# aki-k-no/gaussian-splatting-npu

Hardware: AMD Instinct MI355X
Metric: rendered Mpix/s fwd+bwd, 1M Gaussians @1080p (higher is better)
Workload: dtype f32; 1 GPU; BASELINE config 4: 8 views per step of config 2 (1000000 Gaussians, SH deg 3, 1920x1080, fwd+bwd each), view v on rank v mod 1, grads accumulated on one GPU; P=1000000, width=1920, height=1080, views_per_rank=8, antialiasing=False, parallelism=views-dp1, forward_views_reruns=1

## Files before the change

### gaussian-splatting-npu_amd/csrc/capi.hip

```cpp
#include <stdio.h>
#include <stdlib.h>
#include <string.h>

#include <string>
#include <vector>

#include "gsr.h"
#include "simple_knn.h"
#include "fused_ssim.h"
#include "gsr_common.h"
#include "gsr_kernels.h"

using namespace gsr;

static_assert(GSR_ACC_MEANS3D == ACC_MEANS3D && GSR_ACC_DC == ACC_DC && GSR_ACC_SH == ACC_SH &&
                  GSR_ACC_OPACITY == ACC_OPACITY && GSR_ACC_SCALES == ACC_SCALES &&
                  GSR_ACC_ROTATIONS == ACC_ROTATIONS && GSR_ACC_COV3D == ACC_COV3D && GSR_ACC_COLORS == ACC_COLORS,
              "include/gsr.h accumulate bits match the kernel's");

namespace {

thread_local std::string g_err;
thread_local uint32_t* g_pinned = nullptr;
constexpr uint32_t L_PENDING = 0xFFFFFFFFu;
constexpr int GSR_RERUN_WIDE = -100;
thread_local int t_last_depth_passes[MAX_VIEWS] = {};
// ... 27 lines not shown
    } while (0)

constexpr int PINNED_SLOT_WORDS = 16;
int pinned(int slot, uint32_t** out)
{
    if (!g_pinned) {
        hipError_t e = hipHostMalloc((void**)&g_pinned, 4 * PINNED_SLOT_WORDS * (MAX_VIEWS + 2),
                                     hipHostMallocMapped | hipHostMallocCoherent);
        if (e != hipSuccess) return fail_hip(e, __LINE__);
    }
    *out = g_pinned + PINNED_SLOT_WORDS * slot;
    return GSR_OK;
}

constexpr unsigned EVENT_FLAGS = hipEventDisableTiming | hipEventDisableSystemFence;
struct PrefixStream {
    hipStream_t s = nullptr;
    hipEvent_t in = nullptr, out = nullptr;
};
constexpr int MAX_DEVICES = 64;
thread_local PrefixStream g_prefix[MAX_DEVICES];
thread_local PrefixStream g_aux[MAX_DEVICES];
thread_local int g_prefix_mode = 1;

int stream_fork(PrefixStream* streams, bool on, hipStream_t from, hipStream_t* out)
{
    *out = from;
    if (!on) return GSR_OK;
    int dev = 0;
    HIP_TRY(hipGetDevice(&dev));
    if (dev < 0 || dev >= MAX_DEVICES) return GSR_OK;
    PrefixStream& ps = streams[dev];
    if (!ps.s) {
        int least = 0, greatest = 0;
        HIP_TRY(hipDeviceGetStreamPriorityRange(&least, &greatest));
        HIP_TRY(hipEventCreateWithFlags(&ps.in, EVENT_FLAGS));
        HIP_TRY(hipEventCreateWithFlags(&ps.out, EVENT_FLAGS));
        HIP_TRY(hipStreamCreateWithPriority(&ps.s, hipStreamNonBlocking, greatest));
    }
    HIP_TRY(hipEventRecord(ps.in, from));
    HIP_TRY(hipStreamWaitEvent(ps.s, ps.in, 0));
    *out = ps.s;
    return GSR_OK;
}

int stream_join(PrefixStream* streams, hipStream_t from, hipStream_t forked)
// ... 77 lines not shown
struct Camera {
    const float *view, *proj, *campos;
    float tan_fovx, tan_fovy;
};
struct ViewState {
    char *geometry, *image, *binning;
    size_t binning_capacity;
    float *out_color, *invdepth;
    int* radii;
};

}

extern "C" {

const char* gsr_last_error(void) { return g_err.c_str(); }

const char* gsr_version(void) { return GSR_REF_ALPHA ? "gsr-hip 0.1 gfx950 ref-alpha (TEST BUILD)" : "gsr-hip 0.1 gfx950"; }

int gsr_set_prefix_stream(int on)
{
    if (on < 0 || on > 2) return fail(GSR_ERR_INVALID, "prefix stream mode must be 0, 1 or 2");
    g_prefix_mode = on;
    return GSR_OK;
}

int gsr_profile_enable(int on)
{
    g_prof.on = on != 0;
    for (int k = 0; k < PK_COUNT; k++) g_prof.used[k] = 0;
    return PK_COUNT;
}

const char* gsr_profile_kernel_name(int k) { return (k >= 0 && k < PK_COUNT) ? kProfNames[k] : ""; }

int gsr_profile_read(double* total_ms, int* counts, int n)
{
    for (int k = 0; k < PK_COUNT && k < n; k++) {
        double acc = 0.0;
        for (size_t j = 0; j < g_prof.used[k]; j++) {
            auto& ev = g_prof.pool[k][j];
            HIP_TRY(hipEventSynchronize(ev.second));
            float ms = 0.f;
            HIP_TRY(hipEventElapsedTime(&ms, ev.first, ev.second));
            acc += ms;
        }
// ... 286 lines not shown
    TileHistJob hj[MAX_VIEWS];
    OrderJob dj[MAX_VIEWS];
    for (int v = 0; v < V; v++) {
        char* gb = vs[v].geometry;
        const PreprocessArgs& a = pa[v];
        rec[v] = {a.tiles_touched, at<uint32_t>(gb, g.off[GEOM_EMIT_START]), P, a.scan_status + scan_status_words(P),
                  nullptr};
        dsort[v] = depth_sort_job(gb, a, hdev[v]);
        uint32_t* offsets = at<uint32_t>(gb, g.off[GEOM_POINT_OFFSETS]);
        off[v] = {offsets, offsets, P, a.scan_status, hdev[v] + 2};
        hj[v] = {a.rect4, P, a.tile_diff};
        dj[v] = diff_order_job(vs[v].image, sc.width, sc.height);
    }
    hipStream_t aux = ps;
    int rc = stream_fork(g_aux, g_prefix_mode != 0, ps, &aux);
    if (rc) return rc;
    hipError_t e = launch_scan_batch(rec, V, true, aux);
    if (e == hipSuccess && use_tile_diff(tg.gx, tg.gy)) {
        ProfScope ps_(PK_RANGES, aux);
        e = launch_tile_hist_batch(hj, V, tg.gx, tg.gy, aux);
    }
    if (e == hipSuccess && use_tile_diff(tg.gx, tg.gy)) {
        ProfScope ps_(PK_TILE_ORDER, aux);
        e = launch_tile_order_batch(dj, V, tg.T, aux);
    }
    if (e == hipSuccess) {
        ProfScope ps_(PK_DEPTH_SORT, ps);
        e = radix_sort_batch(dsort, V, DEPTH_BITS, ps);
    }
    if (e == hipSuccess) {
        ProfScope ps_(PK_SCAN, ps);
        e = launch_scan_batch(off, V, false, ps);
    }
    rc = stream_join(g_aux, ps, aux);
    if (e != hipSuccess) return fail_hip(e, __LINE__);
    if (rc) return rc;
    if (opt.early_count) {
        int all[MAX_VIEWS];
        for (int v = 0; v < V; v++) all[v] = v;
        rc = tile_sort_count_pass(sc, vs, all, V, ps);
        if (rc) return rc;
    }
    DEBUG_SYNC(ps);
    int wide[MAX_VIEWS], nw = 0;
    for (int v = 0; v < V && !rc; v++) {
        rc = forward_geometry_wait(h[v], ps, &L[v]);
        t_last_depth_passes[v] = depth_force_wide() ? 4 : 3;
// ... 18 lines not shown
    }
    if (rc)
        for (int v = 0; v < V; v++) L[v] = 0;
    return rc;
}

static int forward_render(const Scene& sc, const ViewState* vs, const int* L, const int* which, int n,
                          const float* background, bool counted, hipStream_t caller, hipStream_t ps, bool debug)
{
    const TileGrid tg(sc.width, sc.height);
    const ImageLayout im = image_layout(sc.width, sc.height);
    TileSortJob tsort[MAX_VIEWS];
    RangesJob rj[MAX_VIEWS];
    OrderJob oj[MAX_VIEWS];
    RenderFwdArgs ra[MAX_VIEWS];
    int ns = 0;
    for (int k = 0; k < n; k++) {
        const ViewState& s = vs[which[k]];
        const int Lv = L[which[k]];
        if (Lv > 0) tsort[ns++] = fused_tile_sort_job(sc, s, Lv, false);
        uint2* ranges = at<uint2>(s.image, im.off[IMG_RANGES]);
        rj[k] = {Lv, Lv > 0 ? at<uint32_t>(s.binning, bin_layout(Lv).off[BIN_SORTED_TILES]) : nullptr, ranges};
        oj[k] = {ranges, nullptr, at<uint32_t>(s.image, im.off[IMG_TILE_ORDER])};
        ra[k] = render_fwd_args(sc, s, Lv, background);
    }
    if (ns) {
        ProfScope ps_(PK_TILE_SORT, ps, counted);
        HIP_TRY(tile_sort_fused_batch(tsort, ns, tg.gx, tg.T, ps, counted ? FUSED_SCATTER : FUSED_ALL));
    }
    DEBUG_SYNC(ps);
    if (n && !use_tile_diff(tg.gx, tg.gy)) {
        {
            ProfScope ps_(PK_RANGES, ps);
            HIP_TRY(launch_tile_ranges_batch(rj, n, tg.T, ps));
        }
        DEBUG_SYNC(ps);
        ProfScope ps_(PK_TILE_ORDER, ps);
        HIP_TRY(launch_tile_order_batch(oj, n, tg.T, ps));
    }
    DEBUG_SYNC(ps);
    const int rc = stream_join(g_prefix, caller, ps);
    if (rc) return rc;
    if (n) {
        ProfScope ps_(PK_RENDER_FWD, caller);
        HIP_TRY(launch_render_fwd_batch(ra, n, tg.T, caller));
    }
    DEBUG_SYNC(caller);
    return GSR_OK;
}

static bool binning_fits(const ViewState& vs, int L)
{
    return vs.binning && gsr_binning_buffer_size(L) <= vs.binning_capacity;
}

int gsr_forward_geometry_dc(char* geometry_buffer, char* image_buffer, int P, int D, int M, int width, int height,
                         const float* means3D, const float* dc, const float* shs, const float* colors_precomp,
                         const float* opacities, const float* scales, float scale_modifier,
                         const float* rotations, const float* cov3D_precomp, const float* viewmatrix,
                         const float* projmatrix, const float* cam_pos, float tan_fovx, float tan_fovy,
                         bool prefiltered, bool antialiasing, int* radii, bool debug, gsr_stream_t stream,
// ... 160 lines not shown
    r.T = tg.T;
    r.bg = background;
    r.splat = at<float4>(gb, g.off[GEOM_SPLAT]);
    r.final_Ts = at<float>(ib, im.off[IMG_FINAL_T]);
    r.n_contrib = at<uint32_t>(ib, im.off[IMG_N_CONTRIB]);
    r.dL_dpixels = dL_dpix;
    r.dL_invdepths = dL_invdepths;
    r.grad_inst = at<float>(bb, b.off[BIN_GRAD_INST]);
    r.slot = slots_from_rect(tg.gx, tg.gy) ? nullptr : at<uint32_t>(bb, b.off[BIN_SLOT]);
    r.valid = at<uint32_t>(bb, b.off[BIN_VALID]);
    r.hit = at<uint8_t>(bb, b.off[BIN_HIT]);
    r.emit_start = at<uint32_t>(gb, g.off[GEOM_EMIT_START]);
    r.rec_mask = at<uint32_t>(gb, g.off[GEOM_REC_MASK]);
    return r;
}

static int backward_render_impl(const Scene& sc, const ViewState& vs, int R, const float* background,
                                const float* dL_dpix, const float* dL_invdepths, bool debug, hipStream_t s)
{
    const ImageLayout im = image_layout(sc.width, sc.height);
    const RenderBwdArgs r = render_bwd_args(sc, vs, R, background, dL_dpix, dL_invdepths);
    {
        ProfScope ps_(PK_TILE_ORDER, s);
        HIP_TRY(launch_tile_order(nullptr, r.tile_work, r.T, at<uint32_t>(vs.image, im.off[IMG_TILE_ORDER]), s));
    }
    {
        ProfScope ps_(PK_RENDER_BWD, s);
        HIP_TRY(launch_render_bwd(r, r.T, s));
    }
    DEBUG_SYNC(s);
    return GSR_OK;
}

static int preprocess_bwd_shared(PreprocessBwdArgs& p, const Scene& sc, bool has_invdepth, float* dL_dcolor,
                                 float* dL_dopacity, float* dL_dmean3D, float* dL_dcov3D, float* dL_ddc,
                                 float* dL_dsh, float* dL_dscale, float* dL_drot, unsigned accumulate)
{
    if (accumulate & ~(unsigned)GSR_ACC_ALL) return fail(GSR_ERR_INVALID, "unknown accumulate bits");
    if (sc.dc && !dL_ddc) return fail(GSR_ERR_INVALID, "dc given without dL_ddc");
    if (sc.dc && sc.colors_precomp)
        return fail(GSR_ERR_INVALID, "Please provide exactly one of either SHs or precomputed colors!");
    if (sc.dc && sc.M > 0 && (!sc.shs || !dL_dsh))
        return fail(GSR_ERR_INVALID, "dc given with M > 0 but shs/dL_dsh NULL");
    p.P = sc.P; p.D = sc.D; p.M = sc.dc ? sc.M + 1 : sc.M;
    p.means3D = sc.means3D; p.radii = nullptr; p.shs = sc.shs; p.dc = sc.dc; p.dL_ddc = sc.dc ? dL_ddc : nullptr;
    p.opacities = sc.opacities; p.scales = sc.scales; p.rotations = sc.rotations;
    p.scale_modifier = sc.scale_modifier;
// ... 216 lines not shown
    A.dL_dview = dL_dviewmatrix; A.dL_dproj = dL_dprojmatrix; A.dL_dcampos = dL_dcampos;
    hipStream_t s = (hipStream_t)stream;
    {
        ProfScope ps_(PK_CAMERA_BWD, s);
        HIP_TRY(launch_camera_bwd_views(A, s));
    }
    DEBUG_SYNC(s);
    return GSR_OK;
}

int gsr_backward_render_views(int V, int P, const int* R, const float* background, int width, int height,
                              char* const* geom_buffers, char* const* binning_buffers, char* const* image_buffers,
                              const float* const* dL_dpix, const float* const* dL_invdepths, bool debug,
                              gsr_stream_t stream)
{
    if (V < 1 || V > MAX_VIEWS) return fail(GSR_ERR_INVALID, "V must be in [1, 16]");
    if (!R || !geom_buffers || !binning_buffers || !image_buffers || !dL_dpix)
        return fail(GSR_ERR_INVALID, "null per-view array");
    const bool has_inv = dL_invdepths != nullptr;
    if (P <= 0) return GSR_OK;
    OrderJob oj[MAX_VIEWS];
    int no = 0;
    const ImageLayout im = image_layout(width, height);
    const int T = TileGrid(width, height).T;
    for (int v = 0; v < V; v++) {
        if (!image_buffers[v]) return fail(GSR_ERR_ALLOC, "null state buffer");
        if (R[v] > 0)
            oj[no++] = {nullptr, at<uint32_t>(image_buffers[v], im.off[IMG_TILE_WORK]),
                        at<uint32_t>(image_buffers[v], im.off[IMG_TILE_ORDER])};
    }
    Scene sc = {};
    sc.P = P; sc.width = width; sc.height = height;
    RenderBwdArgs ra[MAX_VIEWS];
    int nr = 0;
    for (int v = 0; v < V; v++) {
        if (!dL_dpix[v] || (has_inv && !dL_invdepths[v])) return fail(GSR_ERR_INVALID, "null per-view gradient");
        if (R[v] < 0) return fail(GSR_ERR_INVALID, "R must be >= 0");
        if (R[v] == 0) continue;
        if (!geom_buffers[v] || !binning_buffers[v]) return fail(GSR_ERR_ALLOC, "null state buffer");
        const ViewState vs = {geom_buffers[v], image_buffers[v], binning_buffers[v], 0, nullptr, nullptr, nullptr};
        ra[nr++] = render_bwd_args(sc, vs, R[v], background, dL_dpix[v], has_inv ? dL_invdepths[v] : nullptr);
    }
    if (no) {
        ProfScope ps_(PK_TILE_ORDER, (hipStream_t)stream);
        HIP_TRY(launch_tile_order_batch(oj, no, T, (hipStream_t)stream));
    }
    if (nr) {
        ProfScope ps_(PK_RENDER_BWD, (hipStream_t)stream);
        HIP_TRY(launch_render_bwd_batch(ra, nr, T, (hipStream_t)stream));
    }
    DEBUG_SYNC((hipStream_t)stream);
    return GSR_OK;
}

int gsr_backward_views(int V, int P, int D, int M, const int* R, const float* background, int width, int height,
                       const float* means3D, const float* dc, const float* shs, const float* colors_precomp,
                       const float* opacities, const float* scales, float scale_modifier, const float* rotations,
                       const float* cov3D_precomp, const float* const* viewmatrices,
                       const float* const* projmatrices, const float* const* campos, const float* tan_fovx,
                       const float* tan_fovy, const int* const* radii, char* const* geom_buffers,
                       char* const* binning_buffers, char* const* image_buffers, const float* const* dL_dpix,
                       const float* const* dL_invdepths, float* const* dL_dmean2D, float* dL_dcolor,
                       float* dL_dopacity, float* dL_dmean3D, float* dL_dcov3D, float* dL_ddc, float* dL_dsh,
                       float* dL_dscale, float* dL_drot, bool antialiasing, bool debug, unsigned accumulate,
                       gsr_stream_t stream)
{
    const int rc = gsr_backward_render_views(V, P, R, background, width, height, geom_buffers, binning_buffers,
                                             image_buffers, dL_dpix, dL_invdepths, debug, stream);
// ... 543 lines not shown
```

### gaussian-splatting-npu_amd/csrc/gsr_kernels.h

```cpp
#pragma once
#include <hip/hip_runtime.h>
#include <stdint.h>

namespace gsr {

struct PreprocessArgs {
    int P, D, M, W, H;
    const float* means3D;
    const float* scales;
    float scale_modifier;
    const float* rotations;
    const float* opacities;
    const float* shs;
    const float* dc;
    const float* cov3D_precomp;
    const float* colors_precomp;
    const float* view;
    const float* proj;
    const float* campos;
    float tan_fovx, tan_fovy, focal_x, focal_y;
    uint32_t grid_x, grid_y;
    int prefiltered, antialiasing;
    int* radii;
    float* means2D;
// ... 212 lines not shown
    uint2* ranges;
    bool slotless;
};
size_t fused_pass1_scratch_bytes(int P);
enum FusedPhase { FUSED_COUNT = 1, FUSED_SCATTER = 2, FUSED_ALL = 3 };
hipError_t tile_sort_fused_batch(const TileSortJob* jobs, int V, uint32_t gx, int T, hipStream_t s,
                                 int phases = FUSED_ALL);

struct RangesJob {
    int L;
    const uint32_t* sorted_tiles;
    uint2* ranges;
};
hipError_t launch_tile_ranges_batch(const RangesJob* jobs, int V, int T, hipStream_t s);

struct OrderJob {
    const uint2* ranges;
    const uint32_t* work;
    uint32_t* order;
    const int* diff;
    uint2* ranges_out;
    uint32_t grid_x, grid_y;
};
hipError_t launch_tile_order_batch(const OrderJob* jobs, int V, int T, hipStream_t s);

struct TileHistJob {
    const uint32_t* rect4;
    int P;
    int* diff;
};
hipError_t launch_tile_hist_batch(const TileHistJob* jobs, int V, uint32_t grid_x, uint32_t grid_y, hipStream_t s);

hipError_t radix_sort(int n, int nbits, const uint32_t* keys_in, const uint2* pairs, uint32_t* k0, uint32_t* v0,
                      uint32_t* k1, uint32_t* v1, uint32_t* out_x, uint32_t* out_y, uint32_t* sorted_keys,
                      char* scratch, hipStream_t s, const uint2* rects = nullptr, uint2* sorted_rects = nullptr,
                      uint32_t* sorted_counts = nullptr, SortKind kind = SORT_DEPTH);
hipError_t launch_debug_keys(int L, const uint32_t* sorted_tiles, const uint32_t* point_list, const uint32_t* dkeys,
                             uint64_t* keys, hipStream_t s);
hipError_t launch_debug_keys_from_ranges(int T, const uint2* ranges, const uint32_t* point_list, const uint32_t* dkeys,
                                         uint64_t* keys, hipStream_t s);

hipError_t launch_tile_order(const uint2* ranges, const uint32_t* work, int T, uint32_t* order, hipStream_t s);
hipError_t launch_render_bwd(const RenderBwdArgs& a, int T, hipStream_t s);
hipError_t launch_render_fwd_batch(const RenderFwdArgs* a, int V, int T, hipStream_t s);
hipError_t launch_render_bwd_batch(const RenderBwdArgs* a, int V, int T, hipStream_t s);
hipError_t launch_preprocess_bwd_views(const PreprocessBwdViewsArgs& a, hipStream_t s);
hipError_t launch_preprocess_bwd_single(const PreprocessBwdViewsArgs& a, hipStream_t s);

hipError_t launch_ssim_fwd(int planes, int H, int W, float C1, float C2, const float* img1, const float* img2,
                           float* map, float* dA, float* dB, float* dC, hipStream_t s);
hipError_t launch_ssim_bwd(int planes, int H, int W, const float* img1, const float* img2, const float* dmap,
                           const float* dA, const float* dB, const float* dC, float* dimg1, hipStream_t s);

struct PhotoViews {
    const float* gt[MAX_VIEWS];
    int V, C;
};
size_t photo_loss_workspace_bytes(int V, int C, int H, int W);
hipError_t launch_photo_loss_fwd(const PhotoViews& views, int H, int W, float lambda, bool clamp, const float* img,
                                 float* loss, float* dA, float* dB, float* dC, void* workspace, hipStream_t s);
hipError_t launch_photo_loss_bwd(const PhotoViews& views, int H, int W, float lambda, bool clamp, const float* img,
                                 const float* dloss, const float* dA, const float* dB, const float* dC, float* dimg,
                                 hipStream_t s);

struct ViewLossArgs {
// ... 106 lines not shown
```

### gaussian-splatting-npu_amd/csrc/render.hip

```cpp
#include "gsr_common.h"
#include "gsr_kernels.h"
#if GSR_REF_ALPHA
#define GSR_REF_EXP_QUAL static __device__ __forceinline__
#include "gsr_ref_exp.h"
#endif

namespace gsr {

constexpr int BATCH = 256;

__device__ __forceinline__ void quad_pixel(uint32_t tx, uint32_t ty, int tid, uint32_t& px, uint32_t& py)
{
    const int w = tid >> 6, lane = tid & 63;
    px = tx * GSR_BLOCK_X + (w & 1) * 8 + (lane & 7);
    py = ty * GSR_BLOCK_Y + (w >> 1) * 8 + (lane >> 3);
}

__device__ __forceinline__ float box_min_quadform(float a, float b, float c, float dx0, float dx1, float dy0,
                                                  float dy1)
{
    if (dx0 <= 0.f && dx1 >= 0.f && dy0 <= 0.f && dy1 >= 0.f) return 0.f;
    const float ia = __builtin_amdgcn_rcpf(a), ic = __builtin_amdgcn_rcpf(c);
    float m = 3.0e38f;
    {
// ... 49 lines not shown
{
    const float bq = f.kb * dy;
    const float cq = (f.kc * dy) * dy;
    return fma2(fma2((v2f)(f.ka), dx, (v2f)(bq)), dx, (v2f)(cq));
}

#if GSR_REF_ALPHA
__device__ __forceinline__ float ref_power(const float4 co, float dx, float dy)
{
#pragma clang fp contract(off)
    return -0.5f * (co.x * dx * dx + co.z * dy * dy) - co.y * dx * dy;
}
#endif

__device__ __forceinline__ uint32_t wave_max_u32(uint32_t v)
{
#pragma unroll
    for (int d = 32; d >= 1; d >>= 1) v = max(v, (uint32_t)__shfl_xor((int)v, d, 64));
    return v;
}

constexpr int ORDER_BITS = 6;
constexpr int ORDER_PER_THREAD = 8;

enum OrderMode { ORD_WORK = 0, ORD_RANGES = 1, ORD_DIFF = 2 };

__device__ __forceinline__ void wave_line_scan(int* line, int n, int stride, int lane)
{
    int carry = 0;
    for (int i0 = 0; i0 < n; i0 += 64) {
        const int i = i0 + lane;
        int v = i < n ? line[i * stride] : 0;
#pragma unroll
        for (int d = 1; d < 64; d <<= 1) {
            const int y = __shfl_up(v, d, 64);
            if (lane >= d) v += y;
        }
        v += carry;
        if (i < n) line[i * stride] = v;
        carry = __shfl(v, 63, 64);
    }
}

template <int MODE>
__global__ void __launch_bounds__(1024) tile_order_kernel(const ViewBatch<OrderJob> B, int T)
{
    const OrderJob& J = B.v[blockIdx.x];
    const uint2* ranges = J.ranges;
    const uint32_t* work = J.work;
    uint32_t* order = J.order;
    __shared__ uint32_t s_cnt[16][1 << ORDER_BITS];
    __shared__ uint32_t s_order[1024 * ORDER_PER_THREAD];
    __shared__ uint32_t s_max;
    __shared__ int s_d[MODE == ORD_DIFF ? TILE_DIFF_MAX_CELLS : 1];
    const int tid = threadIdx.x, lane = tid & 63, wid = tid >> 6;
    const uint64_t lt = (1ull << lane) - 1ull;
    const uint32_t gx = J.grid_x, sx = J.grid_x + 1;
    if constexpr (MODE == ORD_DIFF) {
        const int gy = (int)J.grid_y, cells = (int)(sx * (J.grid_y + 1));
        for (int c = tid; c < cells; c += 1024) s_d[c] = J.diff[c];
        __syncthreads();
        for (int r = wid; r < gy; r += 16) wave_line_scan(s_d + r * sx, (int)gx, 1, lane);
        __syncthreads();
        for (int x = wid; x < (int)gx; x += 16) wave_line_scan(s_d + x, gy, (int)sx, lane);
        __syncthreads();
        uint32_t c8[ORDER_PER_THREAD], sum = 0;
#pragma unroll
        for (int i = 0; i < ORDER_PER_THREAD; i++) {
            const int t = tid * ORDER_PER_THREAD + i;
            c8[i] = t < T ? (uint32_t)s_d[(uint32_t)t / gx * sx + (uint32_t)t % gx] : 0u;
            sum += c8[i];
        }
        uint32_t inc = sum;
#pragma unroll
        for (int d = 1; d < 64; d <<= 1) {
// ... 6 lines not shown
        for (int q = 0; q < wid; q++) start += s_cnt[0][q];
#pragma unroll
        for (int i = 0; i < ORDER_PER_THREAD; i++) {
            const int t = tid * ORDER_PER_THREAD + i;
            if (t < T) J.ranges_out[t] = c8[i] ? make_uint2(start, start + c8[i]) : make_uint2(0u, 0u);
            start += c8[i];
        }
        __syncthreads();
    }
    auto load_work = [&](int t) -> uint32_t {
        const int tc = min(t, T - 1);
        uint32_t v;
        if constexpr (MODE == ORD_RANGES) {
            const uint2 r = ranges[tc];
            v = r.y - r.x;
        } else if constexpr (MODE == ORD_DIFF) {
            v = (uint32_t)s_d[(uint32_t)tc / gx * sx + (uint32_t)tc % gx];
        } else {
            v = work[tc];
        }
        return t < T ? v : 0u;
    };
    if (tid == 0) s_max = 0;
    for (int t0 = 0; t0 < T; t0 += 1024 * ORDER_PER_THREAD) {
        uint32_t w[ORDER_PER_THREAD];
#pragma unroll
        for (int i = 0; i < ORDER_PER_THREAD; i++) w[i] = load_work(t0 + (i * 16 + wid) * 64 + lane);
        for (int q = tid; q < 16 * (1 << ORDER_BITS); q += 1024) (&s_cnt[0][0])[q] = 0;
        if (t0 == 0) {
            uint32_t mx = 0;
            for (int t = 1024 * ORDER_PER_THREAD + tid; t < T; t += 1024) mx = max(mx, load_work(t));
#pragma unroll
            for (int i = 0; i < ORDER_PER_THREAD; i++) mx = max(mx, w[i]);
            mx = wave_max_u32(mx);
            __syncthreads();
            if (lane == 0) atomicMax(&s_max, mx);
        }
        __syncthreads();
        const float scale = 63.0f / (float)max(s_max, 1u);
        uint32_t cls[ORDER_PER_THREAD], rank[ORDER_PER_THREAD];
#pragma unroll
        for (int i = 0; i < ORDER_PER_THREAD; i++) {
            const int t = t0 + (i * 16 + wid) * 64 + lane;
            cls[i] = 0u;
            rank[i] = 0u;
            if (t0 + (i * 16 + wid) * 64 >= T) continue;
            const uint32_t c = 63u - min((uint32_t)((float)w[i] * scale), 63u);
            cls[i] = c;
            uint64_t peers = __ballot(t < T);
#pragma unroll
            for (int bit = 0; bit < ORDER_BITS; bit++) {
                const uint64_t bal = __ballot((c >> bit) & 1u);
                peers &= ((c >> bit) & 1u) ? bal : ~bal;
            }
            const uint32_t before = s_cnt[wid][c];
            rank[i] = before + (uint32_t)__popcll(peers & lt);
            if (t < T && (peers & lt) == 0ull) s_cnt[wid][c] = before + (uint32_t)__popcll(peers);
            __builtin_amdgcn_wave_barrier();
        }
        __syncthreads();
        {
            uint32_t tot = 0, mine = 0;
#pragma unroll
            for (int q = 0; q < 16; q++) {
                const uint32_t n = s_cnt[q][lane];
                mine += q < wid ? n : 0u;
                tot += n;
            }
            uint32_t inc = tot;
#pragma unroll
            for (int d = 1; d < 64; d <<= 1) {
                const uint32_t y = (uint32_t)__shfl_up((int)inc, d, 64);
                if (lane >= d) inc += y;
            }
            __syncthreads();
            s_cnt[wid][lane] = inc - tot + mine;
        }
        __syncthreads();
#pragma unroll
        for (int i = 0; i < ORDER_PER_THREAD; i++) {
            const int t = t0 + (i * 16 + wid) * 64 + lane;
            if (t < T) s_order[s_cnt[wid][cls[i]] + rank[i]] = (uint32_t)t;
        }
        __syncthreads();
        const int n = min(T - t0, 1024 * ORDER_PER_THREAD);
        for (int q = tid; q < n; q += 1024) order[t0 + q] = s_order[q];
        __syncthreads();
    }
}

__device__ __forceinline__ uint32_t hit_bits(const uint64_t (*s_hitw)[BATCH / 64], int e)
{
    uint32_t h = 0;
#pragma unroll
    for (int w = 0; w < 4; w++) h |= (uint32_t)((s_hitw[w][e >> 6] >> (e & 63)) & 1ull) << w;
    return h;
}

#ifndef GSR_FWD_WAVES
#define GSR_FWD_WAVES 8
#endif
#ifndef GSR_FWD_STATS
#define GSR_FWD_STATS 0
#endif
#if GSR_FWD_STATS
// ... 462 lines not shown
                            } else {
                                t0[2 * h] += pv.x;
                                t0[2 * h + 1] += pv.y;
                            }
                        }
                    }
                }
                const uint32_t slot = es + myslot;
                float* rec = a.grad_inst + (size_t)slot * GRAD_REC;
                float t[GF_NUM];
#pragma unroll
                for (int f = 0; f < GF_NUM; f++) t[f] = t0[f] + t1[f];
#pragma unroll
                for (int h = 0; h < GF_NUM / 2; h++) reinterpret_cast<float2*>(rec)[h] = make_float2(t[2 * h], t[2 * h + 1]);
                const uint32_t local = slot - es;
                if (local < 32u) atomicOr(&a.rec_mask[id], 1u << local);
                else atomicOr(&a.valid[slot >> 5], 1u << (slot & 31u));
            }
            __builtin_amdgcn_wave_barrier();
        }
    }
}

hipError_t launch_tile_order_batch(const OrderJob* jobs, int V, int T, hipStream_t s)
{
    if (T <= 0) return hipSuccess;
    for (int v0 = 0; v0 < V; v0 += VIEW_BATCH) {
        const int nv = min(VIEW_BATCH, V - v0);
        ViewBatch<OrderJob> B;
        B.n = nv;
        for (int v = 0; v < nv; v++) B.v[v] = jobs[v0 + v];
        if (B.v[0].diff) {
            for (int v = 0; v < nv; v++)
                if (!B.v[v].diff || !use_tile_diff(B.v[v].grid_x, B.v[v].grid_y) || B.v[v].grid_x * B.v[v].grid_y != (uint32_t)T)
                    return hipErrorInvalidValue;
            hipLaunchKernelGGL(tile_order_kernel<ORD_DIFF>, dim3((unsigned)nv), dim3(1024), 0, s, B, T);
        } else if (B.v[0].ranges) {
            hipLaunchKernelGGL(tile_order_kernel<ORD_RANGES>, dim3((unsigned)nv), dim3(1024), 0, s, B, T);
        } else {
            hipLaunchKernelGGL(tile_order_kernel<ORD_WORK>, dim3((unsigned)nv), dim3(1024), 0, s, B, T);
        }
        const hipError_t e = hipGetLastError();
        if (e != hipSuccess) return e;
    }
    return hipSuccess;
}

hipError_t launch_tile_order(const uint2* ranges, const uint32_t* work, int T, uint32_t* order, hipStream_t s)
{
    const OrderJob j = {ranges, work, order};
    return launch_tile_order_batch(&j, 1, T, s);
}

hipError_t launch_render_fwd_batch(const RenderFwdArgs* a, int V, int T, hipStream_t s)
{
    if (T <= 0) return hipSuccess;
    for (int v0 = 0; v0 < V; v0 += VIEW_BATCH) {
        ViewBatch<RenderFwdArgs> B;
        B.n = min(VIEW_BATCH, V - v0);
        for (int v = 0; v < B.n; v++) B.v[v] = a[v0 + v];
        hipLaunchKernelGGL(render_fwd_kernel, dim3((unsigned)T, (unsigned)B.n), dim3(256), 0, s, B);
        const hipError_t e = hipGetLastError();
        if (e != hipSuccess) return e;
    }
    return hipSuccess;
}

hipError_t launch_render_bwd_batch(const RenderBwdArgs* a, int V, int T, hipStream_t s)
{
    if (T <= 0) return hipSuccess;
    for (int v0 = 0; v0 < V; v0 += VIEW_BATCH) {
        ViewBatch<RenderBwdArgs> B;
        B.n = min(VIEW_BATCH, V - v0);
        bool inv = false;
// ... 20 lines not shown
```

### gaussian-splatting-npu_amd/diff_gaussian_rasterization/_C.py

```python
import collections
import ctypes
import functools
import math
import os

import torch

_HERE = os.path.dirname(os.path.abspath(__file__))
LIB_PATH = os.path.join(_HERE, "libgsr_hip.so")

_vp, _i, _f, _b, _sz = ctypes.c_void_p, ctypes.c_int, ctypes.c_float, ctypes.c_bool, ctypes.c_size_t


def _load(path=LIB_PATH):
    if not os.path.exists(path):
        raise ImportError(
            f"diff_gaussian_rasterization: native library {path} is missing; build it with "
            "`make -C gaussian-splatting-npu_amd` (or __graft_entry__.build()). There is no CPU fallback.")
    lib = ctypes.CDLL(path)
    for n in ("gsr_last_error", "gsr_version"):
        getattr(lib, n).restype = ctypes.c_char_p
        getattr(lib, n).argtypes = []
    for n in ("gsr_geometry_buffer_size", "gsr_binning_buffer_size"):
        getattr(lib, n).restype = _sz
# ... 42 lines not shown
    lib.gsr_densify_workspace_size.restype = _sz
    lib.gsr_densify_rows_per_workgroup.argtypes = []
    lib.gsr_densify_plan.argtypes = [_i, _vp, ctypes.c_long, _vp, ctypes.c_long, _vp, _vp, _f, _f, _f, _f, _i, _vp,
                                     ctypes.POINTER(_i), _vp]
    lib.gsr_densify_apply.argtypes = [_i, _i, _i, _i, _i, ctypes.POINTER(_i), _i, _i, _i, _vp, _vp, _vp, _vp, _vp, _vp,
                                      _vp, _vp, _vp]
    lib.gsr_union_rows_per_wave.argtypes = []
    lib.gsr_union_workspace_size.argtypes = [_i]
    lib.gsr_union_workspace_size.restype = _sz
    lib.gsr_visibility_pack.argtypes = [_i, _vp, _vp, _vp]
    lib.gsr_union_plan.argtypes = [_i, _i, _vp, _i, ctypes.POINTER(_i), _vp, _vp, _vp, ctypes.POINTER(_i),
                                   ctypes.POINTER(_i), _vp]
    lib.gsr_rows_gather.argtypes = [_i, _i, _i, _i, _i, ctypes.POINTER(_i), _vp, _vp, _vp, _vp]
    lib.gsr_rows_scatter.argtypes = lib.gsr_rows_gather.argtypes
    lib.gsr_debug_sorted_keys.argtypes = [_vp, _vp, _vp, _i, _i, _i, _i, _vp, _vp, _vp, _vp]
    lib.gsr_debug_depth_sort_workspace_size.argtypes = [_i]
    lib.gsr_debug_depth_sort_workspace_size.restype = _sz
    lib.gsr_debug_depth_sort.argtypes = [_vp, _i, _vp, _vp, _vp]
    if hasattr(lib, "gsr_debug_set_depth_wide"):
        lib.gsr_debug_depth_wide.argtypes = []
        lib.gsr_debug_set_depth_wide.argtypes = [_i]
    if hasattr(lib, "gsr_debug_last_depth_passes"):
        lib.gsr_debug_last_depth_passes.argtypes = [_i]
    for n in ("gsr_geometry_layout", "gsr_binning_layout"):
        getattr(lib, n).argtypes = [_i, ctypes.POINTER(_sz), _i]
    lib.gsr_image_layout.argtypes = [_i, _i, ctypes.POINTER(_sz), _i]
    return lib


lib = _load()


def _check(rc):
    if rc != 0:
        raise RuntimeError(f"diff_gaussian_rasterization (HIP): {lib.gsr_last_error().decode()} [status {rc}]")


_contig_cache = {}
_binning_hint = {}
_binning_hint_views = {}
views_reruns = 0


def _binning_capacity(hint):
    return lib.gsr_binning_buffer_size(min(int(hint * 1.25) + 65536, 0x7FFFFFFF)) if hint is not None else 0

# ... 748 lines not shown
    return keys, vals, ranges


def depth_sort(keys):
    n = keys.numel()
    ids = torch.empty((n,), dtype=torch.int32, device=keys.device)
    if n == 0:
        return ids
    ws = torch.empty((lib.gsr_debug_depth_sort_workspace_size(n),), dtype=torch.uint8, device=keys.device)
    keys = keys.contiguous()
    _check(lib.gsr_debug_depth_sort(keys.data_ptr(), n, ids.data_ptr(), ws.data_ptr(),
                                    _stream(keys.device)))
    return ids


def depth_wide():
    return bool(lib.gsr_debug_depth_wide())


def set_depth_wide(on):
    _check(lib.gsr_debug_set_depth_wide(1 if on else 0))


def grad_record_floats():
    return int(lib.gsr_debug_grad_record_floats())


def last_depth_passes(view=0):
    return int(lib.gsr_debug_last_depth_passes(int(view)))


def fusedssim(C1, C2, img1, img2):
    import fused_ssim
    return fused_ssim.fusedssim(C1, C2, img1, img2, train=False)[0]


def fusedssim_backward(C1, C2, img1, img2, opt_grad):
    import fused_ssim
    _, a, b, c = fused_ssim.fusedssim(C1, C2, img1, img2, train=True)
    return fused_ssim.fusedssim_backward(C1, C2, img1, img2, opt_grad, a, b, c)
```

### include/gsr.h

```cpp
#ifndef GSR_H_INCLUDED
#define GSR_H_INCLUDED

#include <stdbool.h>
#include <stddef.h>
#include <stdint.h>

#ifdef __cplusplus
extern "C" {
#endif

typedef void* gsr_stream_t;

typedef char* (*gsr_resize_fn)(void* ctx, size_t bytes);

enum {
    GSR_OK = 0,
    GSR_ERR_INVALID = 1,
    GSR_ERR_HIP = 2,
    GSR_ERR_ALLOC = 3,
    GSR_ERR_PREFILTERED = 4
};

const char* gsr_last_error(void);
const char* gsr_version(void);
// ... 245 lines not shown

int gsr_densify_apply(int P, int P_after, int n_split, int N, int n_groups, const int* Ms, int xyz_group,
                      int scaling_group, int rotation_group, const float* const* src,
                      const float* const* src_m, const float* const* src_v, float* const* dst,
                      float* const* dst_m, float* const* dst_v, const float* samples, const char* workspace,
                      gsr_stream_t stream);

int gsr_union_rows_per_wave(void);
size_t gsr_union_workspace_size(int P);

int gsr_visibility_pack(int P, const float* count, uint32_t* words, gsr_stream_t stream);

int gsr_union_plan(int P, int ranks, const uint32_t* words, int n_bounds, const int* bounds, char* workspace,
                   uint32_t* rows, uint8_t* mask, int* U, int* bound_ranks, gsr_stream_t stream);

int gsr_rows_gather(int P, int U, int u0, int u1, int n_groups, const int* Ms, const float* const* src,
                    const uint32_t* rows, float* compact, gsr_stream_t stream);

int gsr_rows_scatter(int P, int U, int u0, int u1, int n_groups, const int* Ms, float* const* dst,
                     const uint32_t* rows, const float* compact, gsr_stream_t stream);

int gsr_set_prefix_stream(int on);

int gsr_debug_sorted_keys(const char* geometry_buffer, const char* binning_buffer, const char* image_buffer,
                          int P, int num_rendered, int width, int height,
                          uint64_t* keys_out, uint32_t* vals_out, uint32_t* ranges_out,
                          gsr_stream_t stream);

size_t gsr_debug_depth_sort_workspace_size(int n);
int gsr_debug_depth_sort(const uint32_t* keys, int n, uint32_t* out_ids, char* workspace, gsr_stream_t stream);

int gsr_debug_depth_wide(void);
int gsr_debug_set_depth_wide(int on);
int gsr_debug_last_depth_passes(int view);

int gsr_debug_grad_record_floats(void);

int gsr_geometry_layout(int P, size_t* offsets, int n);
int gsr_image_layout(int width, int height, size_t* offsets, int n);
int gsr_binning_layout(int num_rendered, size_t* offsets, int n);

int gsr_profile_enable(int on);
int gsr_profile_read(double* total_ms, int* counts, int n);
const char* gsr_profile_kernel_name(int kernel_id);

#ifdef __cplusplus
// ... 4 lines not shown
```

Measured before the change: 3669 Mpix/s.

## Interleave tile render order across XCDs by spatial bucket

Extends the tile-order kernel's sort key with a 3-bit spatial bucket (4x4 tile blocks hashed mod 8), so that, within each workload class, tiles are placed at order positions whose residue mod 8 matches their bucket. The intent is that round-robin dispatch of render blocks across the MI355X's 8 XCDs sends spatially coherent tiles to the same XCD, improving L2 reuse of Gaussian data, while the order stays heaviest-first. This adds a more complex shared-memory prefix and free-slot redistribution to the ordering kernel, plus a runtime mode switch that is on by default.

```diff
diff --git a/gaussian-splatting-npu_amd/csrc/capi.hip b/gaussian-splatting-npu_amd/csrc/capi.hip
--- a/gaussian-splatting-npu_amd/csrc/capi.hip
+++ b/gaussian-splatting-npu_amd/csrc/capi.hip
@@ -2,6 +2,7 @@
 #include <stdlib.h>
 #include <string.h>
 
+#include <atomic>
 #include <string>
 #include <vector>
 
@@ -75,6 +76,8 @@
 thread_local PrefixStream g_prefix[MAX_DEVICES];
 thread_local PrefixStream g_aux[MAX_DEVICES];
 thread_local int g_prefix_mode = 1;
+std::atomic<int> g_tile_order_mode{1};
+int tile_order_mode() { return g_tile_order_mode.load(std::memory_order_relaxed); }
 
 int stream_fork(PrefixStream* streams, bool on, hipStream_t from, hipStream_t* out)
 {
@@ -198,6 +201,13 @@
 {
     if (on < 0 || on > 2) return fail(GSR_ERR_INVALID, "prefix stream mode must be 0, 1 or 2");
     g_prefix_mode = on;
+    return GSR_OK;
+}
+
+int gsr_set_tile_order_mode(int mode)
+{
+    if (mode < 0 || mode > 1) return fail(GSR_ERR_INVALID, "tile order mode must be 0 or 1");
+    g_tile_order_mode.store(mode, std::memory_order_relaxed);
     return GSR_OK;
 }
 
@@ -530,7 +540,7 @@
     }
     if (e == hipSuccess && use_tile_diff(tg.gx, tg.gy)) {
         ProfScope ps_(PK_TILE_ORDER, aux);
-        e = launch_tile_order_batch(dj, V, tg.T, aux);
+        e = launch_tile_order_batch(dj, V, tg.T, tile_order_mode(), aux);
     }
     if (e == hipSuccess) {
         ProfScope ps_(PK_DEPTH_SORT, ps);
@@ -595,6 +605,7 @@
         uint2* ranges = at<uint2>(s.image, im.off[IMG_RANGES]);
         rj[k] = {Lv, Lv > 0 ? at<uint32_t>(s.binning, bin_layout(Lv).off[BIN_SORTED_TILES]) : nullptr, ranges};
         oj[k] = {ranges, nullptr, at<uint32_t>(s.image, im.off[IMG_TILE_ORDER])};
+        oj[k].grid_x = tg.gx;
         ra[k] = render_fwd_args(sc, s, Lv, background);
     }
     if (ns) {
@@ -609,7 +620,7 @@
         }
         DEBUG_SYNC(ps);
         ProfScope ps_(PK_TILE_ORDER, ps);
-        HIP_TRY(launch_tile_order_batch(oj, n, tg.T, ps));
+        HIP_TRY(launch_tile_order_batch(oj, n, tg.T, tile_order_mode(), ps));
     }
     DEBUG_SYNC(ps);
     const int rc = stream_join(g_prefix, caller, ps);
@@ -816,7 +827,9 @@
     const RenderBwdArgs r = render_bwd_args(sc, vs, R, background, dL_dpix, dL_invdepths);
     {
         ProfScope ps_(PK_TILE_ORDER, s);
-        HIP_TRY(launch_tile_order(nullptr, r.tile_work, r.T, at<uint32_t>(vs.image, im.off[IMG_TILE_ORDER]), s));
+        HIP_TRY(launch_tile_order(nullptr, r.tile_work, r.T, TileGrid(sc.width, sc.height).gx,
+                                  at<uint32_t>(vs.image, im.off[IMG_TILE_ORDER]),
+                                  tile_order_mode(), s));
     }
     {
         ProfScope ps_(PK_RENDER_BWD, s);
@@ -1079,12 +1092,15 @@
     OrderJob oj[MAX_VIEWS];
     int no = 0;
     const ImageLayout im = image_layout(width, height);
-    const int T = TileGrid(width, height).T;
+    const TileGrid tg(width, height);
+    const int T = tg.T;
     for (int v = 0; v < V; v++) {
         if (!image_buffers[v]) return fail(GSR_ERR_ALLOC, "null state buffer");
-        if (R[v] > 0)
-            oj[no++] = {nullptr, at<uint32_t>(image_buffers[v], im.off[IMG_TILE_WORK]),
-                        at<uint32_t>(image_buffers[v], im.off[IMG_TILE_ORDER])};
+        if (R[v] > 0) {
+            oj[no] = {nullptr, at<uint32_t>(image_buffers[v], im.off[IMG_TILE_WORK]),
+                      at<uint32_t>(image_buffers[v], im.off[IMG_TILE_ORDER])};
+            oj[no++].grid_x = tg.gx;
+        }
     }
     Scene sc = {};
     sc.P = P; sc.width = width; sc.height = height;
@@ -1100,7 +1116,7 @@
     }
     if (no) {
         ProfScope ps_(PK_TILE_ORDER, (hipStream_t)stream);
-        HIP_TRY(launch_tile_order_batch(oj, no, T, (hipStream_t)stream));
+        HIP_TRY(launch_tile_order_batch(oj, no, T, tile_order_mode(), (hipStream_t)stream));
     }
     if (nr) {
         ProfScope ps_(PK_RENDER_BWD, (hipStream_t)stream);
diff --git a/gaussian-splatting-npu_amd/csrc/gsr_kernels.h b/gaussian-splatting-npu_amd/csrc/gsr_kernels.h
--- a/gaussian-splatting-npu_amd/csrc/gsr_kernels.h
+++ b/gaussian-splatting-npu_amd/csrc/gsr_kernels.h
@@ -258,7 +258,7 @@
     uint2* ranges_out;
     uint32_t grid_x, grid_y;
 };
-hipError_t launch_tile_order_batch(const OrderJob* jobs, int V, int T, hipStream_t s);
+hipError_t launch_tile_order_batch(const OrderJob* jobs, int V, int T, int xcd, hipStream_t s);
 
 struct TileHistJob {
     const uint32_t* rect4;
@@ -276,7 +276,8 @@
 hipError_t launch_debug_keys_from_ranges(int T, const uint2* ranges, const uint32_t* point_list, const uint32_t* dkeys,
                                          uint64_t* keys, hipStream_t s);
 
-hipError_t launch_tile_order(const uint2* ranges, const uint32_t* work, int T, uint32_t* order, hipStream_t s);
+hipError_t launch_tile_order(const uint2* ranges, const uint32_t* work, int T, uint32_t grid_x, uint32_t* order, int xcd,
+                             hipStream_t s);
 hipError_t launch_render_bwd(const RenderBwdArgs& a, int T, hipStream_t s);
 hipError_t launch_render_fwd_batch(const RenderFwdArgs* a, int V, int T, hipStream_t s);
 hipError_t launch_render_bwd_batch(const RenderBwdArgs* a, int V, int T, hipStream_t s);
diff --git a/gaussian-splatting-npu_amd/csrc/render.hip b/gaussian-splatting-npu_amd/csrc/render.hip
--- a/gaussian-splatting-npu_amd/csrc/render.hip
+++ b/gaussian-splatting-npu_amd/csrc/render.hip
@@ -95,6 +95,15 @@
 
 constexpr int ORDER_BITS = 6;
 constexpr int ORDER_PER_THREAD = 8;
+constexpr int XCD_BITS = 3;
+constexpr int ORDER_KEYS = 1 << (ORDER_BITS + XCD_BITS);
+static_assert((1024 * ORDER_PER_THREAD) % (1 << XCD_BITS) == 0, "a pass starts at XCD residue `phase`");
+
+__device__ __forceinline__ uint32_t tile_bucket(uint32_t t, uint32_t gx)
+{
+    const uint32_t tx = t % gx, ty = t / gx;
+    return ((tx >> 2) + 3u * (ty >> 2)) & 7u;
+}
 
 enum OrderMode { ORD_WORK = 0, ORD_RANGES = 1, ORD_DIFF = 2 };
 
@@ -116,14 +125,16 @@
 }
 
 template <int MODE>
-__global__ void __launch_bounds__(1024) tile_order_kernel(const ViewBatch<OrderJob> B, int T)
+__global__ void __launch_bounds__(1024) tile_order_kernel(const ViewBatch<OrderJob> B, int T, int xcd)
 {
     const OrderJob& J = B.v[blockIdx.x];
     const uint2* ranges = J.ranges;
     const uint32_t* work = J.work;
     uint32_t* order = J.order;
-    __shared__ uint32_t s_cnt[16][1 << ORDER_BITS];
+    __shared__ uint32_t s_cnt[16][ORDER_KEYS];
     __shared__ uint32_t s_order[1024 * ORDER_PER_THREAD];
+    __shared__ uint4 s_key[ORDER_KEYS], s_free[ORDER_KEYS];
+    __shared__ uint32_t s_wsum[ORDER_KEYS / 64];
     __shared__ uint32_t s_max;
     __shared__ int s_d[MODE == ORD_DIFF ? TILE_DIFF_MAX_CELLS : 1];
     const int tid = threadIdx.x, lane = tid & 63, wid = tid >> 6;
@@ -176,11 +187,13 @@
         return t < T ? v : 0u;
     };
     if (tid == 0) s_max = 0;
+    const uint32_t phase = (blockIdx.x * (uint32_t)T) & 7u;
+    auto item_tile = [&](int t0, int i) { return t0 + (xcd ? wid * ORDER_PER_THREAD + i : i * 16 + wid) * 64; };
     for (int t0 = 0; t0 < T; t0 += 1024 * ORDER_PER_THREAD) {
         uint32_t w[ORDER_PER_THREAD];
 #pragma unroll
-        for (int i = 0; i < ORDER_PER_THREAD; i++) w[i] = load_work(t0 + (i * 16 + wid) * 64 + lane);
-        for (int q = tid; q < 16 * (1 << ORDER_BITS); q += 1024) (&s_cnt[0][0])[q] = 0;
+        for (int i = 0; i < ORDER_PER_THREAD; i++) w[i] = load_work(item_tile(t0, i) + lane);
+        for (int q = tid; q < 16 * ORDER_KEYS; q += 1024) (&s_cnt[0][0])[q] = 0;
         if (t0 == 0) {
             uint32_t mx = 0;
             for (int t = 1024 * ORDER_PER_THREAD + tid; t < T; t += 1024) mx = max(mx, load_work(t));
@@ -192,34 +205,37 @@
         }
         __syncthreads();
         const float scale = 63.0f / (float)max(s_max, 1u);
-        uint32_t cls[ORDER_PER_THREAD], rank[ORDER_PER_THREAD];
+        uint32_t key[ORDER_PER_THREAD], rank[ORDER_PER_THREAD];
 #pragma unroll
         for (int i = 0; i < ORDER_PER_THREAD; i++) {
-            const int t = t0 + (i * 16 + wid) * 64 + lane;
-            cls[i] = 0u;
+            const int t = item_tile(t0, i) + lane;
+            key[i] = 0u;
             rank[i] = 0u;
-            if (t0 + (i * 16 + wid) * 64 >= T) continue;
+            if (item_tile(t0, i) >= T) continue;
             const uint32_t c = 63u - min((uint32_t)((float)w[i] * scale), 63u);
-            cls[i] = c;
+            const uint32_t k = (c << XCD_BITS) | (xcd ? tile_bucket((uint32_t)min(t, T - 1), gx) : 0u);
+            key[i] = k;
             uint64_t peers = __ballot(t < T);
 #pragma unroll
-            for (int bit = 0; bit < ORDER_BITS; bit++) {
-                const uint64_t bal = __ballot((c >> bit) & 1u);
-                peers &= ((c >> bit) & 1u) ? bal : ~bal;
+            for (int bit = 0; bit < ORDER_BITS + XCD_BITS; bit++) {
+                const uint64_t bal = __ballot((k >> bit) & 1u);
+                peers &= ((k >> bit) & 1u) ? bal : ~bal;
             }
-            const uint32_t before = s_cnt[wid][c];
+            const uint32_t before = s_cnt[wid][k];
             rank[i] = before + (uint32_t)__popcll(peers & lt);
-            if (t < T && (peers & lt) == 0ull) s_cnt[wid][c] = before + (uint32_t)__popcll(peers);
+            if (t < T && (peers & lt) == 0ull) s_cnt[wid][k] = before + (uint32_t)__popcll(peers);
             __builtin_amdgcn_wave_barrier();
         }
         __syncthreads();
         {
-            uint32_t tot = 0, mine = 0;
-#pragma unroll
-            for (int q = 0; q < 16; q++) {
-                const uint32_t n = s_cnt[q][lane];
-                mine += q < wid ? n : 0u;
-                tot += n;
+            uint32_t tot = 0;
+            if (tid < ORDER_KEYS) {
+#pragma unroll
+                for (int q = 0; q < 16; q++) {
+                    const uint32_t n = s_cnt[q][tid];
+                    s_cnt[q][tid] = tot;
+                    tot += n;
+                }
             }
             uint32_t inc = tot;
 #pragma unroll
@@ -227,14 +243,54 @@
                 const uint32_t y = (uint32_t)__shfl_up((int)inc, d, 64);
                 if (lane >= d) inc += y;
             }
+            if (tid < ORDER_KEYS && lane == 63) s_wsum[wid] = inc;
             __syncthreads();
-            s_cnt[wid][lane] = inc - tot + mine;
+            if (tid < ORDER_KEYS) {
+                uint32_t ex = inc - tot;
+                for (int q = 0; q < wid; q++) ex += s_wsum[q];
+                const uint32_t h = (uint32_t)lane & 7u;
+                const uint32_t S = (uint32_t)__shfl((int)ex, lane & ~7, 64);
+                uint32_t ncls = tot;
+#pragma unroll
+                for (int d = 1; d < 8; d <<= 1) ncls += (uint32_t)__shfl_xor((int)ncls, d, 64);
+                uint32_t p0 = ex, m = tot;
+                if (xcd) {
+                    p0 = S + ((h - phase - S) & 7u);
+                    m = p0 < S + ncls ? (S + ncls - 1u - p0) / 8u + 1u : 0u;
+                }
+                const uint32_t over = tot > m ? tot - m : 0u, fre = m > tot ? m - tot : 0u;
+                uint32_t lo = over, fr = fre;
+#pragma unroll
+                for (int d = 1; d < 8; d <<= 1) {
+                    const uint32_t yl = (uint32_t)__shfl_up((int)lo, d, 64), yf = (uint32_t)__shfl_up((int)fr, d, 64);
+                    if (h >= (uint32_t)d) {
+                        lo += yl;
+                        fr += yf;
+                    }
+                }
+                const uint32_t f0 = fr - fre;
+                s_key[tid] = make_uint4(p0, min(tot, m), lo - over, xcd ? 8u : 1u);
+                s_free[tid] = make_uint4(f0, f0 + fre, p0 + 8u * (tot - f0), 0u);
+            }
         }
         __syncthreads();
 #pragma unroll
         for (int i = 0; i < ORDER_PER_THREAD; i++) {
-            const int t = t0 + (i * 16 + wid) * 64 + lane;
-            if (t < T) s_order[s_cnt[wid][cls[i]] + rank[i]] = (uint32_t)t;
+            const int t = item_tile(t0, i) + lane;
+            if (t >= T) continue;
+            const uint32_t k = key[i];
+            const uint32_t j = s_cnt[wid][k] + rank[i];
+            const uint4 K = s_key[k];
+            uint32_t p = K.x + K.w * j;
+            if (j >= K.y) {
+                const uint32_t e = K.z + (j - K.y);
+#pragma unroll
+                for (uint32_t h = 0; h < 8; h++) {
+                    const uint4 F = s_free[(k & ~7u) + h];
+                    if (e >= F.x && e < F.y) p = F.z + 8u * e;
+                }
+            }
+            s_order[p] = (uint32_t)t;
         }
         __syncthreads();
         const int n = min(T - t0, 1024 * ORDER_PER_THREAD);
@@ -743,23 +799,26 @@
     }
 }
 
-hipError_t launch_tile_order_batch(const OrderJob* jobs, int V, int T, hipStream_t s)
+hipError_t launch_tile_order_batch(const OrderJob* jobs, int V, int T, int xcd, hipStream_t s)
 {
     if (T <= 0) return hipSuccess;
     for (int v0 = 0; v0 < V; v0 += VIEW_BATCH) {
         const int nv = min(VIEW_BATCH, V - v0);
         ViewBatch<OrderJob> B;
         B.n = nv;
-        for (int v = 0; v < nv; v++) B.v[v] = jobs[v0 + v];
+        for (int v = 0; v < nv; v++) {
+            B.v[v] = jobs[v0 + v];
+            if (xcd && B.v[v].grid_x == 0) return hipErrorInvalidValue;
+        }
         if (B.v[0].diff) {
             for (int v = 0; v < nv; v++)
                 if (!B.v[v].diff || !use_tile_diff(B.v[v].grid_x, B.v[v].grid_y) || B.v[v].grid_x * B.v[v].grid_y != (uint32_t)T)
                     return hipErrorInvalidValue;
-            hipLaunchKernelGGL(tile_order_kernel<ORD_DIFF>, dim3((unsigned)nv), dim3(1024), 0, s, B, T);
+            hipLaunchKernelGGL(tile_order_kernel<ORD_DIFF>, dim3((unsigned)nv), dim3(1024), 0, s, B, T, xcd);
         } else if (B.v[0].ranges) {
-            hipLaunchKernelGGL(tile_order_kernel<ORD_RANGES>, dim3((unsigned)nv), dim3(1024), 0, s, B, T);
+            hipLaunchKernelGGL(tile_order_kernel<ORD_RANGES>, dim3((unsigned)nv), dim3(1024), 0, s, B, T, xcd);
         } else {
-            hipLaunchKernelGGL(tile_order_kernel<ORD_WORK>, dim3((unsigned)nv), dim3(1024), 0, s, B, T);
+            hipLaunchKernelGGL(tile_order_kernel<ORD_WORK>, dim3((unsigned)nv), dim3(1024), 0, s, B, T, xcd);
         }
         const hipError_t e = hipGetLastError();
         if (e != hipSuccess) return e;
@@ -767,10 +826,12 @@
     return hipSuccess;
 }
 
-hipError_t launch_tile_order(const uint2* ranges, const uint32_t* work, int T, uint32_t* order, hipStream_t s)
-{
-    const OrderJob j = {ranges, work, order};
-    return launch_tile_order_batch(&j, 1, T, s);
+hipError_t launch_tile_order(const uint2* ranges, const uint32_t* work, int T, uint32_t grid_x, uint32_t* order, int xcd,
+                             hipStream_t s)
+{
+    OrderJob j = {ranges, work, order};
+    j.grid_x = grid_x;
+    return launch_tile_order_batch(&j, 1, T, xcd, s);
 }
 
 hipError_t launch_render_fwd_batch(const RenderFwdArgs* a, int V, int T, hipStream_t s)
diff --git a/gaussian-splatting-npu_amd/diff_gaussian_rasterization/_C.py b/gaussian-splatting-npu_amd/diff_gaussian_rasterization/_C.py
--- a/gaussian-splatting-npu_amd/diff_gaussian_rasterization/_C.py
+++ b/gaussian-splatting-npu_amd/diff_gaussian_rasterization/_C.py
@@ -88,6 +88,8 @@
         lib.gsr_debug_set_depth_wide.argtypes = [_i]
     if hasattr(lib, "gsr_debug_last_depth_passes"):
         lib.gsr_debug_last_depth_passes.argtypes = [_i]
+    if hasattr(lib, "gsr_set_tile_order_mode"):
+        lib.gsr_set_tile_order_mode.argtypes = [_i]
     for n in ("gsr_geometry_layout", "gsr_binning_layout"):
         getattr(lib, n).argtypes = [_i, ctypes.POINTER(_sz), _i]
     lib.gsr_image_layout.argtypes = [_i, _i, ctypes.POINTER(_sz), _i]
@@ -882,6 +884,10 @@
     _check(lib.gsr_debug_set_depth_wide(1 if on else 0))
 
 
+def set_tile_order_mode(mode):
+    _check(lib.gsr_set_tile_order_mode(int(mode)))
+
+
 def grad_record_floats():
     return int(lib.gsr_debug_grad_record_floats())
 
diff --git a/include/gsr.h b/include/gsr.h
--- a/include/gsr.h
+++ b/include/gsr.h
@@ -291,6 +291,8 @@
 
 int gsr_set_prefix_stream(int on);
 
+int gsr_set_tile_order_mode(int mode);
+
 int gsr_debug_sorted_keys(const char* geometry_buffer, const char* binning_buffer, const char* image_buffer,
                           int P, int num_rendered, int width, int height,
                           uint64_t* keys_out, uint32_t* vals_out, uint32_t* ranges_out,
```

After: 3692 Mpix/s, median of 6. About the same (+0.6%).
